# 0x002A/MuCHSALSA

Hardware: AMD Instinct MI355X
Metric: overlap-pairs/s (higher is better)
Workload: dtype int32+f64; 1 GPU; 100k synthetic Nanopore x10 kb, 500k unitig anchors, 10x coverage (BASELINE.json configs[2]); rows=5059558, reads=100000, anchors=499992, edges=981460, edgematches_rank0=25532466, orders_rank0=1029308, parallelism=one job on one GPU, edges_proven_clean_rank0=5372

## Files before the change

### include/msgpu.h

```cpp
#ifndef MSGPU_H
#define MSGPU_H

#include <stddef.h>
#include <stdint.h>

#ifdef __cplusplus
extern "C" {
#endif

#define MSGPU_VERSION 1

#define MSGPU_OK 0
#define MSGPU_E_IO (-1)
#define MSGPU_E_FORMAT (-2)
#define MSGPU_E_NUMBER (-3)
#define MSGPU_E_NOMEM (-4)
#define MSGPU_E_ARG (-5)
#define MSGPU_E_HIP (-6)
#define MSGPU_E_STATE (-7)
#define MSGPU_E_IDS (-8)
#define MSGPU_E_NODEVICE (-9)
#define MSGPU_E_LAYOUT (-10)
#define MSGPU_E_TIMEOUT (-11)

// ... 132 lines not shown
uint32_t    msgpu_paf_anchor_count(const msgpu_paf *paf);
const char *msgpu_paf_read_name(const msgpu_paf *paf, uint32_t read_id);
const char *msgpu_paf_anchor_name(const msgpu_paf *paf, uint32_t anchor_id);

struct msgpu_seqfile;
int msgpu_paf_register_sequences(msgpu_paf *paf, int kind, const struct msgpu_seqfile *f, uint32_t *ids, uint32_t *id_space);

int msgpu_index_lines(const char *path, uint64_t *offsets, size_t capacity, size_t *n_lines);
typedef struct msgpu_registry msgpu_registry;
msgpu_registry *msgpu_registry_new(void);
void     msgpu_registry_free(msgpu_registry *r);
uint32_t msgpu_registry_id(msgpu_registry *r, const char *name);
uint32_t msgpu_registry_size(const msgpu_registry *r);
void     msgpu_registry_clear(msgpu_registry *r);
int      msgpu_toggle_mul(int a, int b);


int msgpu_load_rows(msgpu_ctx *ctx, const msgpu_row *rows, size_t n_rows);
int msgpu_load_rows_packed(msgpu_ctx *ctx, const msgpu_packed_rows *packed);
int msgpu_load_rows_device(msgpu_ctx *ctx, const void *d_rows, size_t n_rows);


int msgpu_calculate_edges(msgpu_ctx *ctx);


int msgpu_chaining_and_overlaps(msgpu_ctx *ctx);


int msgpu_get_counts(msgpu_ctx *ctx, msgpu_counts *out);
int msgpu_get_timings(msgpu_ctx *ctx, msgpu_timings *out);
int msgpu_get_chain_band_counts(msgpu_ctx *ctx, uint64_t *n_banded, uint64_t *n_fallback);
int msgpu_chain_band_width(void);
int msgpu_cand_wide(uint32_t largest_read_cnt);
int msgpu_set_stage_events(msgpu_ctx *ctx, int on);

int msgpu_copy_tables(msgpu_ctx *ctx, msgpu_edge *edges, msgpu_edgematch *ems, msgpu_order *orders, uint32_t *ids);
int msgpu_copy_tables_device(msgpu_ctx *ctx, void *d_edges, void *d_ems, void *d_orders, void *d_ids);
int msgpu_copy_reads(msgpu_ctx *ctx, int32_t *read_len, uint32_t *read_first_line);

int msgpu_merge_gathered(msgpu_ctx *ctx, const void *d_gathered, uint32_t world, const uint64_t *counts,
                         uint64_t slab_bytes, uint64_t off_edges, uint64_t off_orders, uint64_t off_ids, void *d_edges,
                         void *d_orders, void *d_ids);

int msgpu_merge_gathered_ex(msgpu_ctx *ctx, const void *d_gathered, uint32_t world, const uint64_t *counts,
                            uint64_t slab_bytes, uint64_t off_edges, uint64_t off_orders, uint64_t off_ids,
                            const uint32_t *id_base, void *d_edges, void *d_orders, void *d_ids, void *hip_stream);

uint64_t msgpu_wire_edges_bytes(uint64_t n_edges);
uint64_t msgpu_wire_orders_bytes(uint64_t n_orders);
uint64_t msgpu_wire_ids_bytes(uint64_t n_ids, uint32_t id_bytes);
int msgpu_pack_wire(msgpu_ctx *ctx, void *d_wire_edges, void *d_wire_orders, void *d_ids, uint32_t id_bytes);
int msgpu_merge_wire(msgpu_ctx *ctx, const void *d_gathered, uint32_t world, const uint64_t *counts, uint64_t slab_bytes,
                     uint64_t off_edges, uint64_t off_orders, uint64_t off_ids, uint32_t id_bytes, const uint32_t *id_base,
                     void *d_edges, void *d_orders, void *d_ids, void *hip_stream);
int msgpu_unpack_wire_host(const void *wire_edges, const void *wire_orders, const void *wire_ids, uint32_t id_bytes,
                           uint64_t n_edges, uint64_t n_orders, uint64_t n_ids, const uint64_t *base, msgpu_edge *edges,
                           msgpu_order *orders, uint32_t *ids, uint32_t threads, uint32_t tables);

typedef struct msgpu_group msgpu_group;
typedef struct msgpu_group_tables {
  const msgpu_edge  *edges;
  const msgpu_order *orders;
  const uint32_t    *ids;
  const int32_t     *read_len;
  const uint32_t    *read_first_line;
  uint64_t n_edges, n_orders, n_ids, n_ems;
// ... 869 lines not shown
```

### muchsalsa_amd/_lib.py

```python
import ctypes as C
import os

import numpy as np

_HERE = os.path.dirname(os.path.abspath(__file__))
LIB_PATH = os.environ.get("MSGPU_LIB") or os.path.join(_HERE, "libmsgpu.so")

ROW_DTYPE = np.dtype([("anchor_id", "<u4"), ("read_id", "<u4"), ("read_len", "<i4"), ("i_lo", "<i4"),
                      ("i_hi", "<i4"), ("n_lo", "<i4"), ("n_hi", "<i4"), ("score", "<u4"), ("line", "<u4"),
                      ("flags", "<u4")])
EDGE_DTYPE = np.dtype([("v1", "<u4"), ("v2", "<u4"), ("em_off", "<u8"), ("order_off", "<u8"), ("em_cnt", "<u4"),
                       ("order_cnt", "<u2"), ("shadow", "u1"), ("pad", "u1")])
EM_DTYPE = np.dtype([("ov_lo", "<i4"), ("ov_hi", "<i4"), ("score", "<f8"), ("anchor_id", "<u4"), ("line", "<u4"),
                     ("flags", "<u4"), ("edge_idx", "<u4")])
ORDER_DTYPE = np.dtype([("edge_idx", "<u4"), ("flags", "<u4"), ("left_offset", "<f8"), ("right_offset", "<f8"),
                        ("score", "<u8"), ("ids_off", "<u8"), ("ids_cnt", "<u4"), ("start", "<u4"), ("end", "<u4"),
                        ("base", "<u4"), ("pad", "<u4", (2,))])
COPY_DTYPE = np.dtype([("src_off", "<u8"), ("dst_off", "<u8"), ("len", "<u4"), ("flags", "<u4")])
assert (ROW_DTYPE.itemsize, EDGE_DTYPE.itemsize, EM_DTYPE.itemsize, ORDER_DTYPE.itemsize) == (40, 32, 32, 64)
assert COPY_DTYPE.itemsize == 24
COPY_ILLUMINA, COPY_REVCOMP = 1, 2
PATH_READ_DTYPE = np.dtype([("read_id", "<u4"), ("direction", "<u4"), ("nanopore_length", "<u8")])
PATH_ORDER_DTYPE = np.dtype([("score", "<u8"), ("base_read", "<u4"), ("ids_off", "<u4"), ("ids_cnt", "<u4"),
                             ("pad", "<u4")])
# ... 377 lines not shown
EV_TEXT_HEAD, EV_TEXT_REPORT, EV_TEXT_SPECTRUM, EV_TEXT_BED = 0, 1, 2, 3


SYMBOLS = [
    ("msgpu_default_params", None, [C.POINTER(Params)]),
    ("msgpu_strerror", C.c_char_p, [C.c_int]),
    ("msgpu_create", C.c_int, [C.c_int, C.POINTER(Params), C.POINTER(C.c_void_p)]),
    ("msgpu_destroy", None, [C.c_void_p]),
    ("msgpu_last_error", C.c_char_p, [C.c_void_p]),
    ("msgpu_set_stream", C.c_int, [C.c_void_p, C.c_void_p]),
    ("msgpu_get_stream", C.c_void_p, [C.c_void_p]),
    ("msgpu_stream_wait", C.c_int, [C.c_void_p, C.c_void_p]),
    ("msgpu_stream_release", C.c_int, [C.c_void_p, C.c_void_p]),
    ("msgpu_set_shard", C.c_int, [C.c_void_p, C.c_uint32, C.c_uint32]),
    ("msgpu_set_id_space", C.c_int, [C.c_void_p, C.c_uint32, C.c_uint32]),
    ("msgpu_parse_paf", C.c_int, [C.c_char_p, C.POINTER(Params), C.POINTER(C.c_void_p)]),
    ("msgpu_paf_free", None, [C.c_void_p]),
    ("msgpu_paf_rows", C.c_void_p, [C.c_void_p, C.POINTER(C.c_size_t)]),
    ("msgpu_paf_line_count", C.c_size_t, [C.c_void_p]),
    ("msgpu_paf_read_count", C.c_uint32, [C.c_void_p]),
    ("msgpu_paf_anchor_count", C.c_uint32, [C.c_void_p]),
    ("msgpu_paf_read_name", C.c_char_p, [C.c_void_p, C.c_uint32]),
    ("msgpu_paf_anchor_name", C.c_char_p, [C.c_void_p, C.c_uint32]),
    ("msgpu_paf_register_sequences", C.c_int, [C.c_void_p, C.c_int, C.c_void_p, C.c_void_p, C.POINTER(C.c_uint32)]),
    ("msgpu_load_rows", C.c_int, [C.c_void_p, C.c_void_p, C.c_size_t]),
    ("msgpu_load_rows_device", C.c_int, [C.c_void_p, C.c_void_p, C.c_size_t]),
    ("msgpu_calculate_edges", C.c_int, [C.c_void_p]),
    ("msgpu_chaining_and_overlaps", C.c_int, [C.c_void_p]),
    ("msgpu_get_counts", C.c_int, [C.c_void_p, C.POINTER(Counts)]),
    ("msgpu_get_timings", C.c_int, [C.c_void_p, C.POINTER(Timings)]),
    ("msgpu_get_chain_band_counts", C.c_int, [C.c_void_p, C.POINTER(C.c_uint64), C.POINTER(C.c_uint64)]),
    ("msgpu_chain_band_width", C.c_int, []),
    ("msgpu_cand_wide", C.c_int, [C.c_uint32]),
    ("msgpu_set_stage_events", C.c_int, [C.c_void_p, C.c_int]),
    ("msgpu_copy_tables", C.c_int, [C.c_void_p, C.c_void_p, C.c_void_p, C.c_void_p, C.c_void_p]),
    ("msgpu_copy_tables_device", C.c_int, [C.c_void_p, C.c_void_p, C.c_void_p, C.c_void_p, C.c_void_p]),
    ("msgpu_copy_reads", C.c_int, [C.c_void_p, C.c_void_p, C.c_void_p]),
    ("msgpu_merge_gathered", C.c_int, [C.c_void_p, C.c_void_p, C.c_uint32, C.c_void_p, C.c_uint64, C.c_uint64,
                                       C.c_uint64, C.c_uint64, C.c_void_p, C.c_void_p, C.c_void_p]),
    ("msgpu_merge_gathered_ex", C.c_int, [C.c_void_p, C.c_void_p, C.c_uint32, C.c_void_p, C.c_uint64, C.c_uint64,
                                          C.c_uint64, C.c_uint64, C.c_void_p, C.c_void_p, C.c_void_p, C.c_void_p,
                                          C.c_void_p]),
    ("msgpu_wire_edges_bytes", C.c_uint64, [C.c_uint64]),
    ("msgpu_wire_orders_bytes", C.c_uint64, [C.c_uint64]),
    ("msgpu_wire_ids_bytes", C.c_uint64, [C.c_uint64, C.c_uint32]),
    ("msgpu_pack_wire", C.c_int, [C.c_void_p, C.c_void_p, C.c_void_p, C.c_void_p, C.c_uint32]),
    ("msgpu_merge_wire", C.c_int, [C.c_void_p, C.c_void_p, C.c_uint32, C.c_void_p, C.c_uint64, C.c_uint64, C.c_uint64,
                                   C.c_uint64, C.c_uint32, C.c_void_p, C.c_void_p, C.c_void_p, C.c_void_p, C.c_void_p]),
    ("msgpu_chain_launches", C.c_uint64, [C.c_void_p]),
    ("msgpu_wait_chain_launch", C.c_int, [C.c_void_p, C.c_uint64, C.c_uint32]),
    ("msgpu_unpack_wire_host", C.c_int, [C.c_void_p, C.c_void_p, C.c_void_p, C.c_uint32, C.c_uint64, C.c_uint64, C.c_uint64,
                                         C.POINTER(C.c_uint64), C.c_void_p, C.c_void_p, C.c_void_p, C.c_uint32, C.c_uint32]),
    ("msgpu_find_contraction_edges", C.c_int, [C.c_void_p, C.c_void_p, C.c_uint64, C.c_void_p, C.c_uint64, C.c_uint32,
                                               C.c_void_p]),
    ("msgpu_pack_rows", C.c_int, [C.c_void_p, C.c_size_t, C.c_uint32, C.POINTER(PackedRows)]),
    ("msgpu_packed_rows_free", None, [C.POINTER(PackedRows)]),
    ("msgpu_load_rows_packed", C.c_int, [C.c_void_p, C.POINTER(PackedRows)]),
    ("msgpu_synchronize", C.c_int, [C.c_void_p]),
    ("msgpu_set_deadline", C.c_int, [C.c_void_p, C.c_uint32]),
    ("msgpu_debug_buffers", C.c_int, [C.c_void_p, C.c_char_p, C.c_size_t, C.POINTER(C.c_size_t)]),
    ("msgpu_seq_parse", C.c_int, [C.c_char_p, C.c_int, C.POINTER(C.c_void_p)]),
    ("msgpu_seq_free", None, [C.c_void_p]),
    ("msgpu_seq_count", C.c_uint32, [C.c_void_p]),
    ("msgpu_seq_name", C.c_char_p, [C.c_void_p, C.c_uint32]),
    ("msgpu_seq_length", C.c_uint64, [C.c_void_p, C.c_uint32]),
    ("msgpu_seq_bases", C.c_void_p, [C.c_void_p, C.c_uint32]),
# ... 305 lines not shown
```

### muchsalsa_amd/csrc/msgpu_api.hip

```cpp
#include <hip/hip_runtime.h>

#include <chrono>
#include <cmath>
#include <cstdarg>
#include <cstdio>
#include <cstdlib>
#include <cstring>
#include <condition_variable>
#include <deque>
#include <mutex>
#include <new>
#include <thread>
#include <vector>
#include <algorithm>
#include <sys/mman.h>
#include <unistd.h>

#include "asm_internal.h"
#include "host_pool.h"
#include "msgpu.h"
#include "msgpu_internal.h"
#include "msgpu_devbuf.h"
#include "msgpu_stage.h"

// ... 1226 lines not shown
  if (c->stage_events) STAGE_HIP(c, hipEventRecord(c->ev[8], st));
  c->have_chain_t = true;
  c->have_stage_t = c->stage_events;
  c->state        = ST_CHAINED;
  return MSGPU_OK;
}

int msgpu_set_stage_events(msgpu_ctx *c, int on) {
  if (!c) return MSGPU_E_ARG;
  c->stage_events = on != 0;
  return MSGPU_OK;
}

int msgpu_get_counts(msgpu_ctx *c, msgpu_counts *out) {
  if (!c || !out) return MSGPU_E_ARG;
  memset(out, 0, sizeof(*out));
  out->n_rows_in       = c->n_rows;
  out->n_rows_alive    = c->n_alive;
  out->n_reads         = c->V;
  out->n_anchors       = c->A;
  out->n_edges         = c->state >= ST_EDGES ? c->n_edges : 0;
  out->n_ems           = c->state >= ST_EDGES ? c->n_ems : 0;
  out->n_orders        = c->state >= ST_CHAINED ? c->n_orders : 0;
  out->n_ids           = c->state >= ST_CHAINED ? c->n_ids : 0;
  out->n_pairs_scanned = c->state >= ST_EDGES ? c->n_visit : 0;
  out->n_edges_fastpath = c->state >= ST_CHAINED ? c->n_edges_fast : 0;
  out->n_lost_publications = c->sc.lost;
  out->index_path          = c->index_path;
  return MSGPU_OK;
}

int msgpu_chain_band_width(void) { return MSGPU_CHAIN_BAND; }
int msgpu_cand_wide(uint32_t largest_read_cnt) { return cand_wide(largest_read_cnt) ? 1 : 0; }

static int chain_band_counts_impl(msgpu_ctx *c, uint64_t *n_banded, uint64_t *n_fallback);
int msgpu_get_chain_band_counts(msgpu_ctx *c, uint64_t *n_banded, uint64_t *n_fallback) {
  return entry(c, ENTRY_PLAIN, [&] { return chain_band_counts_impl(c, n_banded, n_fallback); });
}
static int chain_band_counts_impl(msgpu_ctx *c, uint64_t *n_banded, uint64_t *n_fallback) {
  if (!c || !n_banded || !n_fallback) return MSGPU_E_ARG;
  *n_banded = *n_fallback = 0;
  if (c->state < ST_CHAINED || !c->chain_chunks.p) return MSGPU_OK;
  STAGE_HIP(c, hipSetDevice(c->device));
  const size_t n_chunks = static_cast<size_t>((c->chain_E + COMPACT_CHUNK - 1) / COMPACT_CHUNK);
  const size_t fb_word  = 2 * static_cast<size_t>(c->chain_E / COMPACT_CHUNK + 1);
  std::vector<unsigned long long> w(fb_word + 1);
  STAGE_HIP(c, hipStreamSynchronize(c->stream));
  STAGE_HIP(c, hipMemcpy(w.data(), c->chain_chunks.p, w.size() * 8, hipMemcpyDeviceToHost));
  for (size_t k = 0; k < n_chunks; ++k) *n_banded += (w[2 * k] >> 16) & 0xffffull;
  *n_fallback = w[fb_word];
  return MSGPU_OK;
}

int msgpu_get_timings(msgpu_ctx *c, msgpu_timings *out) {
  if (!c || !out) return MSGPU_E_ARG;
  memset(out, 0, sizeof(*out));
  STAGE_HIP(c, hipStreamSynchronize(c->stream));
  if (c->have_index_t) STAGE_HIP(c, hipEventElapsedTime(&out->index_ms, c->ev[0], c->ev[1]));
  if (c->have_cand_t) STAGE_HIP(c, hipEventElapsedTime(&out->candidates_ms, c->ev[2], c->ev[3]));
  if (c->have_chain_t) {
    if (c->have_stage_t) {
      STAGE_HIP(c, hipEventElapsedTime(&out->chain_ms, c->ev[4], c->ev[7]));
      STAGE_HIP(c, hipEventElapsedTime(&out->compact_ms, c->ev[7], c->ev[8]));
    }
    double   sum = 0;
    uint32_t n   = 0;
// ... 777 lines not shown
```

### muchsalsa_amd/csrc/msgpu_device.h

```cpp
#ifndef MSGPU_DEVICE_H
#define MSGPU_DEVICE_H

#include <hip/hip_runtime.h>
#include <stdint.h>

#include "msgpu.h"
#include "msgpu_internal.h"

namespace msgpu {

__device__ __forceinline__ IRow load_irow(const IRow *p) {
  const uint4 *q = reinterpret_cast<const uint4 *>(p);
  uint4        a = q[0], b = q[1];
  IRow         r;
  r.n_lo  = static_cast<int>(a.x);
  r.n_hi  = static_cast<int>(a.y);
  r.i_lo  = static_cast<int>(a.z);
  r.i_hi  = static_cast<int>(a.w);
  r.score = b.x;
  r.line  = b.y;
  r.other = b.z;
  r.pf    = b.w;
  return r;
}
// ... 28 lines not shown
  return r;
}
__device__ __forceinline__ void store_srow(SRow *p, const SRow &r) {
  *reinterpret_cast<uint4 *>(p) = make_uint4(static_cast<uint32_t>(r.i_lo), static_cast<uint32_t>(r.i_hi), r.read, r.pf);
}
__device__ __forceinline__ SRow make_srow(const IRow &row, uint32_t read, uint32_t rank) {
  SRow out;
  out.i_lo = row.i_lo;
  out.i_hi = row.i_hi;
  out.read = read;
  out.pf   = (row.pf & ~PF_POS_MASK) | (rank & PF_POS_MASK);
  return out;
}
__device__ __forceinline__ SRow make_srow(const msgpu_row &row, uint32_t read, uint32_t rank) {
  SRow out;
  out.i_lo = row.i_lo;
  out.i_hi = row.i_hi;
  out.read = read;
  out.pf   = ((row.flags & MSGPU_ROW_DIR) ? PF_DIR : 0u) | ((row.flags & MSGPU_ROW_PRIMARY) ? PF_PRIM : 0u) |
           (rank & PF_POS_MASK);
  return out;
}

__device__ __forceinline__ int rl_i32(int v, int lane) { return __builtin_amdgcn_readlane(v, lane); }
__device__ __forceinline__ uint32_t rl_u32(uint32_t v, int lane) {
  return static_cast<uint32_t>(__builtin_amdgcn_readlane(static_cast<int>(v), lane));
}
__device__ __forceinline__ uint64_t rl_u64(uint64_t v, int lane) {
  uint32_t lo = rl_u32(static_cast<uint32_t>(v), lane), hi = rl_u32(static_cast<uint32_t>(v >> 32), lane);
  return (static_cast<uint64_t>(hi) << 32) | lo;
}
__device__ __forceinline__ double rl_f64(double v, int lane) {
  return __longlong_as_double(static_cast<long long>(rl_u64(static_cast<uint64_t>(__double_as_longlong(v)), lane)));
}

__device__ __forceinline__ void publish_to_host(const HostPublish &p, int lane, uint64_t v) {
  if (!p.seq) return;
  if (lane < SC_COUNT) p.host[lane] = v;
  __threadfence_system();
  if (lane == 0) __hip_atomic_store(&p.host[SC_COUNT], p.seq, __ATOMIC_RELEASE, __HIP_MEMORY_SCOPE_SYSTEM);
}

__device__ __forceinline__ double std_max(double a, double b) { return (a < b) ? b : a; }
__device__ __forceinline__ double std_min(double a, double b) { return (b < a) ? b : a; }

__device__ __forceinline__ uint32_t wave_incl_scan(uint32_t v) {
  v += static_cast<uint32_t>(__builtin_amdgcn_update_dpp(0, static_cast<int>(v), 0x111, 0xf, 0xf, false));
  v += static_cast<uint32_t>(__builtin_amdgcn_update_dpp(0, static_cast<int>(v), 0x112, 0xf, 0xf, false));
  v += static_cast<uint32_t>(__builtin_amdgcn_update_dpp(0, static_cast<int>(v), 0x114, 0xf, 0xf, false));
  v += static_cast<uint32_t>(__builtin_amdgcn_update_dpp(0, static_cast<int>(v), 0x118, 0xf, 0xf, false));
  v += static_cast<uint32_t>(__builtin_amdgcn_update_dpp(0, static_cast<int>(v), 0x142, 0xa, 0xf, false));
  v += static_cast<uint32_t>(__builtin_amdgcn_update_dpp(0, static_cast<int>(v), 0x143, 0xc, 0xf, false));
  return v;
}

__device__ __forceinline__ uint64_t wave_incl_scan64(uint32_t v) {
  uint64_t inc = v;
  const int lane = threadIdx.x & 63;
#pragma unroll
  for (int d = 1; d < 64; d <<= 1) {
    const uint64_t t = __shfl_up(inc, d);
    if (lane >= d) inc += t;
  }
  return inc;
}
__device__ __forceinline__ uint32_t wave_sum(uint32_t v) {
// ... 226 lines not shown
```

### muchsalsa_amd/csrc/msgpu_internal.h

```cpp
#ifndef MSGPU_INTERNAL_H
#define MSGPU_INTERNAL_H

#include <hip/hip_runtime.h>
#include <stdint.h>

#include "msgpu.h"

namespace msgpu {

struct IRow {
  int32_t  n_lo, n_hi, i_lo, i_hi;
  uint32_t score, line, other, pf;
};
static_assert(sizeof(IRow) == 32, "IRow must be 32 bytes");
struct SRow {
  int32_t  i_lo, i_hi;
  uint32_t read, pf;
};
static_assert(sizeof(SRow) == 16, "SRow must be 16 bytes");
constexpr uint32_t PF_POS_MASK = 0x3fffffffu;
constexpr uint32_t PF_DIR      = 1u << 30;
constexpr uint32_t PF_PRIM     = 1u << 31;

enum { SC_MAXIDS = 0 , SC_ERR = 1, SC_TOTAL_A = 2, SC_TOTAL_B = 3, SC_TOTAL_C = 4, SC_NLISTS = 5 ,
       SC_NBIG = 7, SC_NALIVE = 8, SC_IXFLAGS = 9, SC_BIGSTATS = 10 , SC_BIGCUR = 12 ,
       SC_CLS = 14 ,
       SC_HEADS = 16 , SC_DONE = 17 ,
       SC_OWN = 18 ,
       SC_MAXCNT = 19 , SC_COUNT = 20 };
static_assert(SC_COUNT <= 64, "one wavefront publishes the whole scalar block (publish_to_host)");
struct HostPublish {
  uint64_t *host;
  uint64_t  seq;
};

struct CandDesc {
  uint32_t r, rb, n1, bound;
  uint64_t co, pad;
};
static_assert(sizeof(CandDesc) == 32, "CandDesc must be 32 bytes");

struct ChainDesc {
  uint32_t e, v1, v2, em_cnt;
  uint64_t em_off, cand;
};
static_assert(sizeof(ChainDesc) == 32, "ChainDesc must be 32 bytes");

constexpr uint32_t CAND_RANK_MAX = 65535, CAND_RANK_SURE = 256;
inline bool cand_wide(uint32_t largest_read_cnt) { return largest_read_cnt > CAND_RANK_MAX; }

struct CandArgs {
  const uint32_t *read_off, *read_cnt, *anchor_off;
  const IRow     *by_read;
  const SRow     *by_anchor;
  const uint4    *vis;
  const uint64_t *cand_off;
  uint32_t       *cand_j;
  uint32_t       *cand_q;
  int             cand_wide;
  uint32_t       *edge_scr_v2;
  uint32_t       *edge_scr_start;
  uint32_t       *n_cand, *n_edge;
  unsigned long long *big_stats;
  uint32_t        th_overlap;
};
constexpr uint32_t CAND_CHUNK = 256;
struct CandZero {
  uint32_t *n_cand, *n_edge;
  uint32_t *scalar_words;
  uint32_t  n_scalar_words;
};
struct EmitArgs {
  const uint32_t *n_edge, *n_cand;
  const uint64_t *cand_off;
  const uint32_t *edge_scr_v2, *edge_scr_start;
  uint32_t        V;
  const uint32_t *hist;
  const unsigned long long *chunk_sums;
  uint32_t        n_chunks;
  msgpu_edge     *edges;
  uint64_t       *edge_cand;
  ChainDesc      *desc;
// ... 241 lines not shown
```

### muchsalsa_amd/csrc/msgpu_kernels.hip

```cpp
#include <hip/hip_runtime.h>
#include <stdint.h>
#include <stdlib.h>

#include <type_traits>
#include <utility>

#include "msgpu.h"
#include "msgpu_internal.h"
#include "msgpu_device.h"

namespace msgpu {


constexpr int SCAN_ITEMS = 8;
uint32_t      scan_blocks(uint64_t n);

template <class T> __global__ __launch_bounds__(256) void k_scan_reduce(const uint32_t *in, uint64_t n, T *block_sums) {
  __shared__ T s[4];
  uint64_t     base = static_cast<uint64_t>(blockIdx.x) * 256 * SCAN_ITEMS;
  T            sum  = 0;
  for (int i = 0; i < SCAN_ITEMS; ++i) {
    uint64_t idx = base + static_cast<uint64_t>(i) * 256 + threadIdx.x;
    if (idx < n) sum += in[idx];
  }
// ... 1374 lines not shown
    f.abort_     = rovl & (f.pos | (f.neg & ~um2));
  } else {
    const M rovl = __ballot(k_rlo <= l_rhi) & __ballot(l_rlo <= k_rhi);
    const M u2   = __ballot(k_rlo < l_rlo) & __ballot(k_rhi < l_rhi);
    const M um2  = __ballot(k_rlo > l_rlo) & __ballot(k_rhi > l_rhi);
    f.abort_     = rovl & ((f.neg & ~um2) | (f.pos & ~u2));
  }
  return f;
}

__device__ __forceinline__ int paths_of_direction(unsigned long long act, bool direction, int lane, double pop,
                                                  uint64_t pm, bool em_prim, uint32_t j1, uint32_t q2, uint32_t n1,
                                                  uint32_t n2, double alt_frac, PathRec *paths) {
  if (act == 0) return 0;
  const bool mine = (act >> lane) & 1ull;
  const double best = group_max_f64<64>(mine ? pop : -1.0);
  double maxv;
  int    maxi;
  if (best > 0.0) {
    maxv = best;
    maxi = __builtin_ctzll(__ballot(mine && pop == best));
  } else {
    maxv = 0.0;
    maxi = __builtin_ctzll(act);
  }
  maxi = __builtin_amdgcn_readfirstlane(maxi);
  const unsigned long long prim_lanes = __ballot(mine && em_prim);
  int                      np         = 0;
  const uint64_t           m          = rl_u64(pm, maxi);
  bool                     hp         = (m & prim_lanes) != 0;
  hp |= __popcll(m) > 2;
  if (lane == 0) {
    paths[0].mask    = m;
    paths[0].score   = static_cast<uint64_t>(maxv);
    paths[0].primary = hp;
  }
  np = 1;
  const double       thr  = maxv * alt_frac;
  uint64_t           used = m;
  unsigned long long cand = __ballot(mine && pop > thr);
  while (true) {
    cand &= __ballot((pm & used) == 0);
    if (!cand) break;
    const int      p  = __builtin_ctzll(cand);
    const uint64_t mp = rl_u64(pm, p);
    const double   sp = rl_f64(pop, p);
    if (lane == 0) {
      paths[np].mask    = mp;
      paths[np].score   = static_cast<uint64_t>(sp);
      paths[np].primary = (mp & prim_lanes) != 0;
    }
    ++np;
    used |= mp;
    cand &= ~(1ull << p);
  }
  if (np == 1 && hp) {
    const int first = __builtin_ctzll(m), last = 63 - __builtin_clzll(m);
    const uint32_t qe = direction ? q2 : (n2 - 1 - q2);
    const uint32_t jf = rl_u32(j1, first), jl = rl_u32(j1, last), qf = rl_u32(qe, first), ql = rl_u32(qe, last);
    bool           demote;
    if ((jf != 0 && qf != 0) || (jl != n1 - 1 && ql != n2 - 1)) {
      demote = true;
    } else {
      const bool     on   = (m >> lane) & 1ull;
      const uint64_t below = m & ((1ull << lane) - 1);
      const int      prev  = below ? 63 - __builtin_clzll(below) : lane;
      const uint32_t pj = __shfl(j1, prev), pq = __shfl(qe, prev);
      const bool     firstt = below == 0;
      const uint32_t i_t    = firstt ? 0u : pj + 1u;
      const uint32_t jj_t   = firstt ? 0u : pq + 1u;
      const bool     viol   = on && qe < jj_t;
      const unsigned long long vmask = __ballot(viol);
      const int      fv   = vmask ? __builtin_ctzll(vmask) : 64;
      const bool     i1   = j1 > i_t;
      const bool     i2   = lane < fv ? (qe > jj_t) : (lane == fv ? (n2 > jj_t) : false);
      demote              = __ballot(on && i1 && i2) != 0;
    }
    if (demote && lane == 0) paths[0].primary = 0;
  }
  return np;
}

// ... 323 lines not shown
    len_p  = static_cast<uint32_t>(__popcll(ppl[lane].mask));
    k_p    = true;
  }
  const bool has_primary = __ballot((k_m && prim_m) || (k_p && prim_p)) != 0;
  if (has_primary) {
    k_m = k_m && prim_m;
    k_p = k_p && prim_p;
  }
  const bool has_multi = __ballot((k_m && len_m > 1) || (k_p && len_p > 1)) != 0;
  if (has_multi) {
    k_m = k_m && len_m > 1;
    k_p = k_p && len_p > 1;
  }
  const unsigned long long keep_m = __ballot(k_m), keep_p = __ballot(k_p);
  const int                combined = __popcll(keep_m) + __popcll(keep_p);
  bool                     shadow;
  if (combined > 1) {
    shadow = true;
  } else {
    uint32_t pr = keep_m ? rl_u32(prim_m, __builtin_ctzll(keep_m)) : rl_u32(prim_p, __builtin_ctzll(keep_p));
    shadow      = !pr;
  }

  uint32_t n_orders = 0, n_ids = 0;
  for (int pass = 0; pass < 2; ++pass) {
    unsigned long long keep = pass == 0 ? keep_m : keep_p;
    const PathRec     *pv   = pass == 0 ? pmn : ppl;
    const bool         dir  = pass == 1;
    while (keep) {
      const int pi = __builtin_ctzll(keep);
      keep &= keep - 1;
      const uint64_t mask = pv[pi].mask;
      const int      f = __builtin_ctzll(mask), l = 63 - __builtin_clzll(mask);
      const double   L1 = rl_f64(clo1, f), R1 = rl_f64(ovr1, l);
      double         L2 = rl_f64(clo2, f), R2 = rl_f64(ovr2, l);
      if (!dir) {
        L2 = rl_f64(ovr2, f);
        R2 = rl_f64(clo2, l);
      }
      bool     have = false;
      uint32_t fl   = 0;
      double   lo = 0, ro = 0;
      if (L1 <= L2 && R1 <= R2) {
        have = true;
        fl   = MSGPU_ORD_START_V1 | MSGPU_ORD_CONTAINED;
        lo   = L2 - L1;
        ro   = R2 - R1;
      } else if (L1 >= L2 && R1 >= R2) {
        have = true;
        fl   = MSGPU_ORD_CONTAINED;
        lo   = L1 - L2;
        ro   = R1 - R2;
      } else if (L1 > L2 && R1 < R2) {
        have = true;
        fl   = MSGPU_ORD_START_V1;
        lo   = L1 - L2;
        ro   = R2 - R1;
      } else if (L1 < L2 && R1 > R2) {
        have = true;
        fl   = 0;
        lo   = L2 - L1;
        ro   = R1 - R2;
      }
      if (!have) continue;
      const uint32_t cnt = static_cast<uint32_t>(__popcll(mask));
      if ((mask >> lane) & 1ull) {
        const uint32_t pos = static_cast<uint32_t>(__popcll(mask & ((1ull << lane) - 1)));
        a.ids_scr[ed.em_off + n_ids + pos] = anchor;
      }
      if (lane == 0) {
        msgpu_order o;
        o.edge_idx     = static_cast<uint32_t>(e);
        o.flags        = fl | (dir ? MSGPU_ORD_DIR : 0u) | (pv[pi].primary ? MSGPU_ORD_PRIMARY : 0u);
        o.left_offset  = lo;
        o.right_offset = ro;
        o.score        = pv[pi].score;
        o.ids_off      = n_ids;
        o.ids_cnt      = cnt;
        o.start        = (fl & MSGPU_ORD_START_V1) ? v1 : v2;
        o.end          = (fl & MSGPU_ORD_START_V1) ? v2 : v1;
        o.base         = v1;
        o.pad[0]       = 0;
        o.pad[1]       = 0;
        a.order_scr[ed.em_off + n_orders] = o;
      }
      ++n_orders;
      n_ids += cnt;
    }
  }
  if (lane == 0) {
    edge_counts(a.edges, e, n, n_orders, n_ids, shadow);
    chunk_add(a.chunk_sums, e, clean, n_orders, n_ids, banded);
  }
}
__global__ __launch_bounds__(64) __attribute__((amdgpu_waves_per_eu(8, 8))) void k_chain(ChainArgs a, const ChainDesc *desc, uint32_t n_desc) {
  chain_body<true, false>(a, desc, n_desc);
}
__global__ __launch_bounds__(64) __attribute__((amdgpu_waves_per_eu(8, 8))) void k_chain_wide(ChainArgs a, const ChainDesc *desc, uint32_t n_desc) {
  chain_body<true, true>(a, desc, n_desc);
}
template <bool WIDE>
__global__ __launch_bounds__(64) __attribute__((amdgpu_waves_per_eu(8, 8))) void k_chain_unlisted(ChainArgs a) {
  chain_body<false, WIDE>(a, nullptr, 0u);
}


struct __attribute__((aligned(16))) SubPath {
  uint32_t mask, primary;
  uint64_t score;
};

__device__ __forceinline__ double shfl_f64(double v, int src) {
  const long long b  = __double_as_longlong(v);
  const uint32_t  lo = __shfl(static_cast<uint32_t>(b), src), hi = __shfl(static_cast<uint32_t>(b >> 32), src);
  return __longlong_as_double(static_cast<long long>((static_cast<unsigned long long>(hi) << 32) | lo));
}

template <int W> __device__ __forceinline__ uint32_t group_bits(unsigned long long m, int gbase) {
// ... 25 lines not shown
    const uint32_t r  = row_bcast<K - 16>(v);
    const uint32_t ro = static_cast<uint32_t>(__builtin_amdgcn_mov_dpp(static_cast<int>(v), 0x150 + K - 16, 0xa, 0xf, false));
    return __builtin_amdgcn_permlane16_swap(r, ro, false, false)[1];
  }
}
template <int W, int K> __device__ __forceinline__ double group_bcast_f64(double v) {
  const unsigned long long b  = __builtin_bit_cast(unsigned long long, v);
  const uint32_t           lo = group_bcast<W, K>(static_cast<uint32_t>(b));
  const uint32_t           hi = group_bcast<W, K>(static_cast<uint32_t>(b >> 32));
  return __builtin_bit_cast(double, (static_cast<unsigned long long>(hi) << 32) | lo);
}

template <typename F, int... K> __device__ __forceinline__ void unroll_while(F &&f, std::integer_sequence<int, K...>) {
  (void)(f(std::integral_constant<int, K>{}) && ...);
}

template <int W>
__device__ __forceinline__ uint32_t paths_of_direction_sub(uint32_t act, bool direction, int sl, int gbase, double pop,
                                                           uint32_t pm, bool em_prim, uint32_t j1, uint32_t q2,
                                                           uint32_t n1, uint32_t n2, double alt_frac, SubPath *paths) {
  const bool live = act != 0;
  const bool mine = (act >> sl) & 1u;
  const double best = group_max_f64<W>(mine ? pop : -1.0);
  double maxv = 0.0;
  int    maxi = live ? __builtin_ctz(act) : 0;
  if (best > 0.0) {
    maxv = best;
    const uint32_t at = group_bits<W>(__ballot(mine && pop == best), gbase);
    maxi = at ? __builtin_ctz(at) : 0;
  }
  const uint32_t prim_lanes = group_bits<W>(__ballot(mine && em_prim), gbase);
  const uint32_t m          = __shfl(pm, gbase + maxi);
  const bool     hp         = ((m & prim_lanes) != 0) | (__popc(m) > 2);
  if (live && sl == 0) paths[0] = SubPath{m, hp ? 1u : 0u, static_cast<uint64_t>(maxv)};
  uint32_t np = live ? 1u : 0u;
  const double thr  = maxv * alt_frac;
  uint32_t     used = m;
  uint32_t     cand = group_bits<W>(__ballot(mine && pop > thr), gbase);
  while (true) {
    cand &= group_bits<W>(__ballot((pm & used) == 0), gbase);
    if (__ballot(cand != 0) == 0) break;
    const bool     has = cand != 0;
    const int      p   = has ? __builtin_ctz(cand) : 0;
    const uint32_t mp  = __shfl(pm, gbase + p);
    const double   sp  = shfl_f64(pop, gbase + p);
    if (has && sl == 0) paths[np] = SubPath{mp, (mp & prim_lanes) != 0 ? 1u : 0u, static_cast<uint64_t>(sp)};
    if (has) {
      ++np;
      used |= mp;
      cand &= ~(1u << p);
    }
  }
  const bool     single = live && np == 1 && hp;
  const uint32_t ms     = m ? m : 1u;
  const int      first = __builtin_ctz(ms), last = 31 - __builtin_clz(ms);
  const uint32_t qe = direction ? q2 : (n2 - 1 - q2);
  const uint32_t jf = __shfl(j1, gbase + first), jl = __shfl(j1, gbase + last);
  const uint32_t qf = __shfl(qe, gbase + first), ql = __shfl(qe, gbase + last);
  const bool     ends   = (jf != 0 && qf != 0) || (jl != n1 - 1 && ql != n2 - 1);
  const bool     on     = (m >> sl) & 1u;
  const uint32_t below  = m & ((1u << sl) - 1u);
  const int      prev   = below ? 31 - __builtin_clz(below) : sl;
  const uint32_t pj = __shfl(j1, gbase + prev), pq = __shfl(qe, gbase + prev);
  const bool     firstt = below == 0;
  const uint32_t i_t = firstt ? 0u : pj + 1u, jj_t = firstt ? 0u : pq + 1u;
  const bool     viol  = on && qe < jj_t;
  const uint32_t vmask = group_bits<W>(__ballot(viol), gbase);
  const int      fv    = vmask ? __builtin_ctz(vmask) : 64;
  const bool     i1    = j1 > i_t;
  const bool     i2    = sl < fv ? (qe > jj_t) : (sl == fv ? (n2 > jj_t) : false);
  const bool     inter = group_bits<W>(__ballot(on && i1 && i2), gbase) != 0;
  if (single && (ends || inter) && sl == 0) paths[0].primary = 0;
  return np;
}

template <int W, bool WIDE>
__device__ __forceinline__ void chain_sub_body(const ChainArgs &a, const ChainDesc *list, uint32_t n_list, uint32_t block,
                                               unsigned char (*s_wavebuf)[sizeof(ChainElem) * 64], uint32_t (*s_cm)[64],
                                               double (*s_keep)[64][4], uint32_t (*s_anchor)[64]) {
// ... 283 lines not shown
  __builtin_amdgcn_fence(__ATOMIC_RELEASE, "wavefront");
  __builtin_amdgcn_wave_barrier();

  bool     k_m = false, k_p = false;
  uint32_t prim_m = 0, prim_p = 0, len_m = 0, len_p = 0;
  if (sl < static_cast<int>(n_m)) {
    prim_m = pmn[sl].primary;
    len_m  = static_cast<uint32_t>(__popc(pmn[sl].mask));
    k_m    = true;
  }
  if (sl < static_cast<int>(n_p)) {
    prim_p = ppl[sl].primary;
    len_p  = static_cast<uint32_t>(__popc(ppl[sl].mask));
    k_p    = true;
  }
  const bool has_primary = group_bits<W>(__ballot((k_m && prim_m) || (k_p && prim_p)), gbase) != 0;
  if (has_primary) {
    k_m = k_m && prim_m;
    k_p = k_p && prim_p;
  }
  const bool has_multi = group_bits<W>(__ballot((k_m && len_m > 1) || (k_p && len_p > 1)), gbase) != 0;
  if (has_multi) {
    k_m = k_m && len_m > 1;
    k_p = k_p && len_p > 1;
  }
  const uint32_t keep_m = group_bits<W>(__ballot(k_m), gbase), keep_p = group_bits<W>(__ballot(k_p), gbase);
  const int      combined = __popc(keep_m) + __popc(keep_p);
  bool           shadow   = true;
  if (combined == 1) shadow = !(keep_m ? pmn[__builtin_ctz(keep_m)].primary : ppl[__builtin_ctz(keep_p)].primary);

  uint32_t n_orders = 0, n_ids = 0;
  {
    uint32_t km = keep_m, kp = keep_p;
    while (__ballot((km | kp) != 0)) {
      const bool     dir  = km == 0;
      const uint32_t keep = dir ? kp : km;
      const bool     has  = keep != 0;
      const int      pi   = has ? __builtin_ctz(keep) : 0;
      km &= km - 1u;
      kp = dir ? (keep & (keep - 1u)) : kp;
      const SubPath  rec  = (dir ? ppl : pmn)[pi];
      const uint32_t mask = (has && rec.mask) ? rec.mask : 1u;
      const int      f = __builtin_ctz(mask), l = 31 - __builtin_clz(mask);
      const double  *kf = s_keep[wave][gbase + f], *kl = s_keep[wave][gbase + l];
      const double   L1 = kf[0], R1 = kl[2];
      const double   L2 = dir ? kf[1] : kf[3], R2 = dir ? kl[3] : kl[1];
      bool     have = false;
      uint32_t fl   = 0;
      double   lo = 0, ro = 0;
      if (L1 <= L2 && R1 <= R2) {
        have = true;
        fl   = MSGPU_ORD_START_V1 | MSGPU_ORD_CONTAINED;
        lo   = L2 - L1;
        ro   = R2 - R1;
      } else if (L1 >= L2 && R1 >= R2) {
        have = true;
        fl   = MSGPU_ORD_CONTAINED;
        lo   = L1 - L2;
        ro   = R1 - R2;
      } else if (L1 > L2 && R1 < R2) {
        have = true;
        fl   = MSGPU_ORD_START_V1;
        lo   = L1 - L2;
        ro   = R2 - R1;
      } else if (L1 < L2 && R1 > R2) {
        have = true;
        fl   = 0;
        lo   = L2 - L1;
        ro   = R1 - R2;
      }
      const bool emit = has && have;
      if (emit) {
        const uint32_t cnt = static_cast<uint32_t>(__popc(mask));
        if ((mask >> sl) & 1u) a.ids_scr[ed.em_off + n_ids + static_cast<uint32_t>(__popc(mask & ((1u << sl) - 1u)))] = s_anchor[wave][lane];
        if (sl == 0) {
          msgpu_order o;
          o.edge_idx     = e;
          o.flags        = fl | (dir ? MSGPU_ORD_DIR : 0u) | (rec.primary ? MSGPU_ORD_PRIMARY : 0u);
          o.left_offset  = lo;
          o.right_offset = ro;
          o.score        = rec.score;
          o.ids_off      = n_ids;
          o.ids_cnt      = cnt;
          o.start        = (fl & MSGPU_ORD_START_V1) ? v1 : v2;
          o.end          = (fl & MSGPU_ORD_START_V1) ? v2 : v1;
          o.base         = v1;
          o.pad[0]       = 0;
          o.pad[1]       = 0;
          a.order_scr[ed.em_off + n_orders] = o;
        }
        ++n_orders;
        n_ids += cnt;
      }
    }
  }
  if (n && sl == 0) {
    edge_counts(a.edges, e, n, n_orders, n_ids, shadow);
    chunk_add(a.chunk_sums, e, clean, n_orders, n_ids);
  }
}

template <int W, bool WIDE>
__global__ __launch_bounds__(256) __attribute__((amdgpu_waves_per_eu(W == 32 ? 7 : 6, W == 32 ? 7 : 6))) void k_chain_sub(ChainArgs a, const ChainDesc *list, uint32_t n_list) {
  __shared__ __attribute__((aligned(16))) unsigned char s_wavebuf[4][sizeof(ChainElem) * 64];
  __shared__ uint32_t                                  s_cm[4][64];
  __shared__ __attribute__((aligned(16))) double       s_keep[4][64][4];
  __shared__ uint32_t                                  s_anchor[4][64];
  chain_sub_body<W, WIDE>(a, list, n_list, blockIdx.x, s_wavebuf, s_cm, s_keep, s_anchor);
}
#ifndef MSGPU_SUB_WAVES
#define MSGPU_SUB_WAVES 7
#endif
template <bool WIDE>
__device__ __forceinline__ void chain_sub_all_body(const ChainArgs &a, const ChainSubLists &l) {
  __shared__ __attribute__((aligned(16))) unsigned char s_wavebuf[4][sizeof(ChainElem) * 64];
  __shared__ uint32_t                                  s_cm[4][64];
  __shared__ __attribute__((aligned(16))) double       s_keep[4][64][4];
  __shared__ uint32_t                                  s_anchor[4][64];
  uint32_t b = blockIdx.x;
  if (b < l.nb32) {
    chain_sub_body<32, WIDE>(a, l.list32, l.n32, b, s_wavebuf, s_cm, s_keep, s_anchor);
  } else if ((b -= l.nb32) < l.nb16) {
    chain_sub_body<16, WIDE>(a, l.list16, l.n16, b, s_wavebuf, s_cm, s_keep, s_anchor);
// ... 577 lines not shown
      bi += s_w[1][w];
    }
    s_ob[threadIdx.x] = bo;
    s_ib[threadIdx.x] = bi;
    s_em[threadIdx.x] = em;
    if (threadIdx.x == COMPACT_CHUNK - 1) {
      s_ob[COMPACT_CHUNK] = bo + no;
      s_ib[COMPACT_CHUNK] = bi + ni;
    }
    if (my_e < a.n_edges) {
      const uint64_t oo = base_o + bo + a.out_order_base;
      reinterpret_cast<uint4 *>(&a.edges[my_e])[1] = make_uint4(static_cast<uint32_t>(oo), static_cast<uint32_t>(oo >> 32), my_hi.z, my_hi.w);
      if (a.out_em_base) a.edges[my_e].em_off = em + a.out_em_base;
    }
  }
  __syncthreads();
  const uint32_t n_o = s_ob[COMPACT_CHUNK], n_i = s_ib[COMPACT_CHUNK];
  constexpr uint32_t ORD_U = 4, IDS_U = 8;
  if (n_o) {
    const uint32_t sub = threadIdx.x & 3, sl = threadIdx.x >> 2;
    for (uint32_t s0 = 0;;) {
      const uint32_t rem = n_o - s0;
      uint4          w[ORD_U];
      uint32_t       ib[ORD_U];
#pragma unroll
      for (uint32_t k = 0; k < ORD_U; ++k) {
        const uint32_t s  = s0 + min(k * (COMPACT_CHUNK / 4) + sl, rem - 1);
        const uint32_t le = compact_find(s_ob, s);
        w[k]  = reinterpret_cast<const uint4 *>(&a.order_scr[s_em[le] + (s - s_ob[le])])[sub];
        ib[k] = s_ib[le];
      }
#pragma unroll
      for (uint32_t k = 0; k < ORD_U; ++k) {
        const uint32_t off = k * (COMPACT_CHUNK / 4) + sl;
        if (sub == 0) w[k].x += a.out_edge_base;
        if (sub == 2) {
          const uint64_t gio = a.out_ids_base + base_i + ib[k] + w[k].x;
          w[k].x = static_cast<uint32_t>(gio);
          w[k].y = static_cast<uint32_t>(gio >> 32);
        }
        if (off < rem) reinterpret_cast<uint4 *>(&a.orders[base_o + s0 + off])[sub] = w[k];
      }
      if (rem <= ORD_U * (COMPACT_CHUNK / 4)) break;
      s0 += ORD_U * (COMPACT_CHUNK / 4);
    }
  }
  if (n_i) {
    for (uint32_t q0 = 0;;) {
      const uint32_t rem = n_i - q0;
      uint32_t       v[IDS_U];
#pragma unroll
      for (uint32_t k = 0; k < IDS_U; ++k) {
        const uint32_t q  = q0 + min(k * COMPACT_CHUNK + threadIdx.x, rem - 1);
        const uint32_t le = compact_find(s_ib, q);
        v[k] = a.ids_scr[s_em[le] + (q - s_ib[le])];
      }
#pragma unroll
      for (uint32_t k = 0; k < IDS_U; ++k) {
        const uint32_t off = k * COMPACT_CHUNK + threadIdx.x;
        if (off < rem) a.ids[base_i + q0 + off] = v[k];
      }
      if (rem <= IDS_U * COMPACT_CHUNK) break;
      q0 += IDS_U * COMPACT_CHUNK;
    }
  }
}

// ... 376 lines not shown
```

Before: 485.7 million overlap-pairs/s.

## Defer order flag and offset computation from chain kernels to compaction pass

The chain kernels now write raw orders: endpoint coordinates, the score bits and a raw marker flag, all stored from the lanes that own them. The branchy containment classification that needed cross-lane reads of coordinates is moved out of these kernels. The compaction kernel reassembles each 64-byte order across a lane quad with DPP broadcasts and runs a shared branchless order_finish helper to produce the final flags, offsets and start/end. This is meant to cut per-path shuffles and lane-0 serial work in the chain kernels, at the cost of extra ALU work in compaction. Orders with no valid relation are now dropped only on NaN, which may change which orders are emitted compared with the old branch checks.

```diff
diff --git a/include/msgpu.h b/include/msgpu.h
--- a/include/msgpu.h
+++ b/include/msgpu.h
@@ -188,6 +188,8 @@
 int msgpu_get_chain_band_counts(msgpu_ctx *ctx, uint64_t *n_banded, uint64_t *n_fallback);
 int msgpu_chain_band_width(void);
 int msgpu_cand_wide(uint32_t largest_read_cnt);
+int msgpu_order_finish(uint32_t raw_flags, double score, double L1, double L2, double R1, double R2, uint32_t v1, uint32_t v2,
+                       msgpu_order *out);
 int msgpu_set_stage_events(msgpu_ctx *ctx, int on);
 
 int msgpu_copy_tables(msgpu_ctx *ctx, msgpu_edge *edges, msgpu_edgematch *ems, msgpu_order *orders, uint32_t *ids);
diff --git a/muchsalsa_amd/_lib.py b/muchsalsa_amd/_lib.py
--- a/muchsalsa_amd/_lib.py
+++ b/muchsalsa_amd/_lib.py
@@ -433,6 +433,8 @@
     ("msgpu_get_chain_band_counts", C.c_int, [C.c_void_p, C.POINTER(C.c_uint64), C.POINTER(C.c_uint64)]),
     ("msgpu_chain_band_width", C.c_int, []),
     ("msgpu_cand_wide", C.c_int, [C.c_uint32]),
+    ("msgpu_order_finish", C.c_int, [C.c_uint32, C.c_double, C.c_double, C.c_double, C.c_double, C.c_double, C.c_uint32,
+                                     C.c_uint32, C.c_void_p]),
     ("msgpu_set_stage_events", C.c_int, [C.c_void_p, C.c_int]),
     ("msgpu_copy_tables", C.c_int, [C.c_void_p, C.c_void_p, C.c_void_p, C.c_void_p, C.c_void_p]),
     ("msgpu_copy_tables_device", C.c_int, [C.c_void_p, C.c_void_p, C.c_void_p, C.c_void_p, C.c_void_p]),
diff --git a/muchsalsa_amd/csrc/msgpu_api.hip b/muchsalsa_amd/csrc/msgpu_api.hip
--- a/muchsalsa_amd/csrc/msgpu_api.hip
+++ b/muchsalsa_amd/csrc/msgpu_api.hip
@@ -1282,6 +1282,20 @@
 
 int msgpu_chain_band_width(void) { return MSGPU_CHAIN_BAND; }
 int msgpu_cand_wide(uint32_t largest_read_cnt) { return cand_wide(largest_read_cnt) ? 1 : 0; }
+int msgpu_order_finish(uint32_t raw_flags, double score, double L1, double L2, double R1, double R2, uint32_t v1, uint32_t v2,
+                       msgpu_order *out) {
+  const OrderFinish o = order_finish(raw_flags, score, L1, L2, R1, R2, v1, v2);
+  if (out) {
+    out->flags        = o.flags;
+    out->left_offset  = o.lo;
+    out->right_offset = o.ro;
+    out->score        = o.score;
+    out->start        = o.start;
+    out->end          = o.end;
+    out->base         = o.base;
+  }
+  return o.have ? 1 : 0;
+}
 
 static int chain_band_counts_impl(msgpu_ctx *c, uint64_t *n_banded, uint64_t *n_fallback);
 int msgpu_get_chain_band_counts(msgpu_ctx *c, uint64_t *n_banded, uint64_t *n_fallback) {
diff --git a/muchsalsa_amd/csrc/msgpu_device.h b/muchsalsa_amd/csrc/msgpu_device.h
--- a/muchsalsa_amd/csrc/msgpu_device.h
+++ b/muchsalsa_amd/csrc/msgpu_device.h
@@ -84,6 +84,38 @@
 }
 __device__ __forceinline__ double rl_f64(double v, int lane) {
   return __longlong_as_double(static_cast<long long>(rl_u64(static_cast<uint64_t>(__double_as_longlong(v)), lane)));
+}
+
+template <int K> __device__ __forceinline__ uint32_t quad_bcast(uint32_t v) {
+  static_assert(K >= 0 && K < 4, "quad lane");
+  return static_cast<uint32_t>(__builtin_amdgcn_mov_dpp(static_cast<int>(v), K * 0x55, 0xf, 0xf, false));
+}
+
+struct OrderFinish {
+  bool     have;
+  uint32_t flags;
+  double   lo, ro;
+  uint64_t score;
+  uint32_t start, end, base;
+};
+__host__ __device__ inline OrderFinish order_finish(uint32_t raw_flags, double score, double L1, double L2, double R1, double R2,
+                                                    uint32_t v1, uint32_t v2) {
+  const bool c1 = (L1 <= L2) & (R1 <= R2);
+  const bool c2 = !c1 & (L1 >= L2) & (R1 >= R2);
+  const bool c3 = !c1 & !c2 & (L1 > L2) & (R1 < R2);
+  const bool c4 = !c1 & !c2 & !c3 & (L1 < L2) & (R1 > R2);
+  OrderFinish    o;
+  o.have            = c1 | c2 | c3 | c4;
+  const uint32_t fl = c1 ? (MSGPU_ORD_START_V1 | MSGPU_ORD_CONTAINED) : c2 ? MSGPU_ORD_CONTAINED : c3 ? MSGPU_ORD_START_V1 : 0u;
+  const double   dl = L2 - L1, dl_ = L1 - L2, dr = R2 - R1, dr_ = R1 - R2;
+  o.lo    = (c1 | c4) ? dl : (c2 | c3) ? dl_ : 0.0;
+  o.ro    = (c1 | c3) ? dr : (c2 | c4) ? dr_ : 0.0;
+  o.flags = fl | (raw_flags & (MSGPU_ORD_DIR | MSGPU_ORD_PRIMARY));
+  o.score = static_cast<uint64_t>(score);
+  o.start = (fl & MSGPU_ORD_START_V1) ? v1 : v2;
+  o.end   = (fl & MSGPU_ORD_START_V1) ? v2 : v1;
+  o.base  = v1;
+  return o;
 }
 
 __device__ __forceinline__ void publish_to_host(const HostPublish &p, int lane, uint64_t v) {
diff --git a/muchsalsa_amd/csrc/msgpu_internal.h b/muchsalsa_amd/csrc/msgpu_internal.h
--- a/muchsalsa_amd/csrc/msgpu_internal.h
+++ b/muchsalsa_amd/csrc/msgpu_internal.h
@@ -48,6 +48,9 @@
 
 constexpr uint32_t CAND_RANK_MAX = 65535, CAND_RANK_SURE = 256;
 inline bool cand_wide(uint32_t largest_read_cnt) { return largest_read_cnt > CAND_RANK_MAX; }
+
+constexpr uint32_t ORD_RAW = 1u << 31;
+static_assert((ORD_RAW & (MSGPU_ORD_START_V1 | MSGPU_ORD_CONTAINED | MSGPU_ORD_DIR | MSGPU_ORD_PRIMARY)) == 0, "the marker is no flag");
 
 struct CandArgs {
   const uint32_t *read_off, *read_cnt, *anchor_off;
diff --git a/muchsalsa_amd/csrc/msgpu_kernels.hip b/muchsalsa_amd/csrc/msgpu_kernels.hip
--- a/muchsalsa_amd/csrc/msgpu_kernels.hip
+++ b/muchsalsa_amd/csrc/msgpu_kernels.hip
@@ -1430,7 +1430,7 @@
   hp |= __popcll(m) > 2;
   if (lane == 0) {
     paths[0].mask    = m;
-    paths[0].score   = static_cast<uint64_t>(maxv);
+    paths[0].score   = __builtin_bit_cast(uint64_t, maxv);
     paths[0].primary = hp;
   }
   np = 1;
@@ -1445,7 +1445,7 @@
     const double   sp = rl_f64(pop, p);
     if (lane == 0) {
       paths[np].mask    = mp;
-      paths[np].score   = static_cast<uint64_t>(sp);
+      paths[np].score   = __builtin_bit_cast(uint64_t, sp);
       paths[np].primary = (mp & prim_lanes) != 0;
     }
     ++np;
@@ -1835,58 +1835,22 @@
       keep &= keep - 1;
       const uint64_t mask = pv[pi].mask;
       const int      f = __builtin_ctzll(mask), l = 63 - __builtin_clzll(mask);
-      const double   L1 = rl_f64(clo1, f), R1 = rl_f64(ovr1, l);
-      double         L2 = rl_f64(clo2, f), R2 = rl_f64(ovr2, l);
-      if (!dir) {
-        L2 = rl_f64(ovr2, f);
-        R2 = rl_f64(clo2, l);
-      }
-      bool     have = false;
-      uint32_t fl   = 0;
-      double   lo = 0, ro = 0;
-      if (L1 <= L2 && R1 <= R2) {
-        have = true;
-        fl   = MSGPU_ORD_START_V1 | MSGPU_ORD_CONTAINED;
-        lo   = L2 - L1;
-        ro   = R2 - R1;
-      } else if (L1 >= L2 && R1 >= R2) {
-        have = true;
-        fl   = MSGPU_ORD_CONTAINED;
-        lo   = L1 - L2;
-        ro   = R1 - R2;
-      } else if (L1 > L2 && R1 < R2) {
-        have = true;
-        fl   = MSGPU_ORD_START_V1;
-        lo   = L1 - L2;
-        ro   = R2 - R1;
-      } else if (L1 < L2 && R1 > R2) {
-        have = true;
-        fl   = 0;
-        lo   = L2 - L1;
-        ro   = R1 - R2;
-      }
-      if (!have) continue;
+      const double   myL2 = dir ? clo2 : ovr2, myR2 = dir ? ovr2 : clo2;
+      if (__ballot((lane == f && __builtin_isunordered(clo1, myL2)) || (lane == l && __builtin_isunordered(ovr1, myR2))) != 0) continue;
       const uint32_t cnt = static_cast<uint32_t>(__popcll(mask));
       if ((mask >> lane) & 1ull) {
         const uint32_t pos = static_cast<uint32_t>(__popcll(mask & ((1ull << lane) - 1)));
         a.ids_scr[ed.em_off + n_ids + pos] = anchor;
       }
+      uint4 *slot4 = reinterpret_cast<uint4 *>(&a.order_scr[ed.em_off + n_orders]);
       if (lane == 0) {
-        msgpu_order o;
-        o.edge_idx     = static_cast<uint32_t>(e);
-        o.flags        = fl | (dir ? MSGPU_ORD_DIR : 0u) | (pv[pi].primary ? MSGPU_ORD_PRIMARY : 0u);
-        o.left_offset  = lo;
-        o.right_offset = ro;
-        o.score        = pv[pi].score;
-        o.ids_off      = n_ids;
-        o.ids_cnt      = cnt;
-        o.start        = (fl & MSGPU_ORD_START_V1) ? v1 : v2;
-        o.end          = (fl & MSGPU_ORD_START_V1) ? v2 : v1;
-        o.base         = v1;
-        o.pad[0]       = 0;
-        o.pad[1]       = 0;
-        a.order_scr[ed.em_off + n_orders] = o;
-      }
+        const uint64_t sc = pv[pi].score;
+        slot4[0] = make_uint4(static_cast<uint32_t>(e), ORD_RAW | (dir ? MSGPU_ORD_DIR : 0u) | (pv[pi].primary ? MSGPU_ORD_PRIMARY : 0u),
+                              static_cast<uint32_t>(sc), static_cast<uint32_t>(sc >> 32));
+        slot4[2] = make_uint4(n_ids, v1, cnt, v2);
+      }
+      if (lane == f) reinterpret_cast<double2 *>(slot4)[1] = make_double2(clo1, myL2);
+      if (lane == l) reinterpret_cast<double2 *>(slot4)[3] = make_double2(ovr1, myR2);
       ++n_orders;
       n_ids += cnt;
     }
@@ -1978,7 +1942,7 @@
   const uint32_t prim_lanes = group_bits<W>(__ballot(mine && em_prim), gbase);
   const uint32_t m          = __shfl(pm, gbase + maxi);
   const bool     hp         = ((m & prim_lanes) != 0) | (__popc(m) > 2);
-  if (live && sl == 0) paths[0] = SubPath{m, hp ? 1u : 0u, static_cast<uint64_t>(maxv)};
+  if (live && sl == 0) paths[0] = SubPath{m, hp ? 1u : 0u, __builtin_bit_cast(uint64_t, maxv)};
   uint32_t np = live ? 1u : 0u;
   const double thr  = maxv * alt_frac;
   uint32_t     used = m;
@@ -1990,7 +1954,7 @@
     const int      p   = has ? __builtin_ctz(cand) : 0;
     const uint32_t mp  = __shfl(pm, gbase + p);
     const double   sp  = shfl_f64(pop, gbase + p);
-    if (has && sl == 0) paths[np] = SubPath{mp, (mp & prim_lanes) != 0 ? 1u : 0u, static_cast<uint64_t>(sp)};
+    if (has && sl == 0) paths[np] = SubPath{mp, (mp & prim_lanes) != 0 ? 1u : 0u, __builtin_bit_cast(uint64_t, sp)};
     if (has) {
       ++np;
       used |= mp;
@@ -2340,6 +2304,7 @@
   uint32_t n_orders = 0, n_ids = 0;
   {
     uint32_t km = keep_m, kp = keep_p;
+    const double *own = s_keep[wave][lane];
     while (__ballot((km | kp) != 0)) {
       const bool     dir  = km == 0;
       const uint32_t keep = dir ? kp : km;
@@ -2350,53 +2315,20 @@
       const SubPath  rec  = (dir ? ppl : pmn)[pi];
       const uint32_t mask = (has && rec.mask) ? rec.mask : 1u;
       const int      f = __builtin_ctz(mask), l = 31 - __builtin_clz(mask);
-      const double  *kf = s_keep[wave][gbase + f], *kl = s_keep[wave][gbase + l];
-      const double   L1 = kf[0], R1 = kl[2];
-      const double   L2 = dir ? kf[1] : kf[3], R2 = dir ? kl[3] : kl[1];
-      bool     have = false;
-      uint32_t fl   = 0;
-      double   lo = 0, ro = 0;
-      if (L1 <= L2 && R1 <= R2) {
-        have = true;
-        fl   = MSGPU_ORD_START_V1 | MSGPU_ORD_CONTAINED;
-        lo   = L2 - L1;
-        ro   = R2 - R1;
-      } else if (L1 >= L2 && R1 >= R2) {
-        have = true;
-        fl   = MSGPU_ORD_CONTAINED;
-        lo   = L1 - L2;
-        ro   = R1 - R2;
-      } else if (L1 > L2 && R1 < R2) {
-        have = true;
-        fl   = MSGPU_ORD_START_V1;
-        lo   = L1 - L2;
-        ro   = R2 - R1;
-      } else if (L1 < L2 && R1 > R2) {
-        have = true;
-        fl   = 0;
-        lo   = L2 - L1;
-        ro   = R1 - R2;
-      }
-      const bool emit = has && have;
+      const double   myL2 = dir ? own[1] : own[3], myR2 = dir ? own[3] : own[1];
+      const bool     nan_ = (sl == f && __builtin_isunordered(own[0], myL2)) || (sl == l && __builtin_isunordered(own[2], myR2));
+      const bool     emit = has && group_bits<W>(__ballot(nan_), gbase) == 0;
       if (emit) {
         const uint32_t cnt = static_cast<uint32_t>(__popc(mask));
         if ((mask >> sl) & 1u) a.ids_scr[ed.em_off + n_ids + static_cast<uint32_t>(__popc(mask & ((1u << sl) - 1u)))] = s_anchor[wave][lane];
+        uint4 *slot4 = reinterpret_cast<uint4 *>(&a.order_scr[ed.em_off + n_orders]);
         if (sl == 0) {
-          msgpu_order o;
-          o.edge_idx     = e;
-          o.flags        = fl | (dir ? MSGPU_ORD_DIR : 0u) | (rec.primary ? MSGPU_ORD_PRIMARY : 0u);
-          o.left_offset  = lo;
-          o.right_offset = ro;
-          o.score        = rec.score;
-          o.ids_off      = n_ids;
-          o.ids_cnt      = cnt;
-          o.start        = (fl & MSGPU_ORD_START_V1) ? v1 : v2;
-          o.end          = (fl & MSGPU_ORD_START_V1) ? v2 : v1;
-          o.base         = v1;
-          o.pad[0]       = 0;
-          o.pad[1]       = 0;
-          a.order_scr[ed.em_off + n_orders] = o;
+          slot4[0] = make_uint4(e, ORD_RAW | (dir ? MSGPU_ORD_DIR : 0u) | (rec.primary ? MSGPU_ORD_PRIMARY : 0u),
+                                static_cast<uint32_t>(rec.score), static_cast<uint32_t>(rec.score >> 32));
+          slot4[2] = make_uint4(n_ids, v1, cnt, v2);
         }
+        if (sl == f) reinterpret_cast<double2 *>(slot4)[1] = make_double2(own[0], myL2);
+        if (sl == l) reinterpret_cast<double2 *>(slot4)[3] = make_double2(own[2], myR2);
         ++n_orders;
         n_ids += cnt;
       }
@@ -3040,7 +2972,27 @@
       }
 #pragma unroll
       for (uint32_t k = 0; k < ORD_U; ++k) {
+        if (k * (COMPACT_CHUNK / 4) >= rem) break;
         const uint32_t off = k * (COMPACT_CHUNK / 4) + sl;
+        {
+          const uint32_t rf = quad_bcast<0>(w[k].y);
+          const uint32_t s_lo = quad_bcast<0>(w[k].z), s_hi = quad_bcast<0>(w[k].w);
+          const uint32_t a0 = quad_bcast<1>(w[k].x), a1 = quad_bcast<1>(w[k].y), a2 = quad_bcast<1>(w[k].z), a3 = quad_bcast<1>(w[k].w);
+          const uint32_t r1 = quad_bcast<2>(w[k].y), r2 = quad_bcast<2>(w[k].w);
+          const uint32_t b0 = quad_bcast<3>(w[k].x), b1 = quad_bcast<3>(w[k].y), b2 = quad_bcast<3>(w[k].z), b3 = quad_bcast<3>(w[k].w);
+          const bool        raw = (rf & ORD_RAW) != 0;
+          const OrderFinish o = order_finish(rf, raw ? __hiloint2double(static_cast<int>(s_hi), static_cast<int>(s_lo)) : 0.0,
+                                             __hiloint2double(static_cast<int>(a1), static_cast<int>(a0)),
+                                             __hiloint2double(static_cast<int>(a3), static_cast<int>(a2)),
+                                             __hiloint2double(static_cast<int>(b1), static_cast<int>(b0)),
+                                             __hiloint2double(static_cast<int>(b3), static_cast<int>(b2)), r1, r2);
+          const unsigned long long lo = __builtin_bit_cast(unsigned long long, o.lo), ro = __builtin_bit_cast(unsigned long long, o.ro);
+          const uint4 fin = sub == 0   ? make_uint4(w[k].x, o.flags, static_cast<uint32_t>(lo), static_cast<uint32_t>(lo >> 32))
+                            : sub == 1 ? make_uint4(static_cast<uint32_t>(ro), static_cast<uint32_t>(ro >> 32), static_cast<uint32_t>(o.score), static_cast<uint32_t>(o.score >> 32))
+                            : sub == 2 ? make_uint4(w[k].x, 0u, w[k].z, o.start)
+                                       : make_uint4(o.end, o.base, 0u, 0u);
+          w[k] = make_uint4(raw ? fin.x : w[k].x, raw ? fin.y : w[k].y, raw ? fin.z : w[k].z, raw ? fin.w : w[k].w);
+        }
         if (sub == 0) w[k].x += a.out_edge_base;
         if (sub == 2) {
           const uint64_t gio = a.out_ids_base + base_i + ib[k] + w[k].x;
```

Measured after the change: 491.1 million overlap-pairs/s, median of 6. +1.1%, better.
